# wh-xu/Hyper-Gen

Measured on AMD Instinct MI355X. Metric: genomes/sec sketch (k=21,s=1500,D=4096), higher is better.
Workload: dtype u64

## Files before the change

### hyper-gen_amd/csrc/hg_encode_kernels.hip

```cpp
#include "hg_internal.h"

namespace {

constexpr int ENC_WG = 512;
constexpr int ENC_WAVES = ENC_WG / 64;
constexpr uint64_t WY_INC = 0xa0761d6478bd642full;
constexpr uint64_t WY_XOR = 0xe7037ed1a0b428dbull;

__device__ __forceinline__ uint64_t wy_word(uint64_t hash, uint64_t off) {
  uint64_t s = hash + off;
  unsigned __int128 m = (unsigned __int128)(s ^ WY_XOR) * s;
  return (uint64_t)(m >> 64) ^ (uint64_t)m;
}

__device__ __forceinline__ void csa(uint64_t &hi, uint64_t &lo, uint64_t a, uint64_t b, uint64_t c) {
  const uint32_t a0 = (uint32_t)a, a1 = (uint32_t)(a >> 32), b0 = (uint32_t)b, b1 = (uint32_t)(b >> 32);
  const uint32_t c0 = (uint32_t)c, c1 = (uint32_t)(c >> 32);
  const uint32_t h0 = __builtin_amdgcn_bitop3_b32(a0, b0, c0, 0xE8), h1 = __builtin_amdgcn_bitop3_b32(a1, b1, c1, 0xE8);
  const uint32_t l0 = __builtin_amdgcn_bitop3_b32(a0, b0, c0, 0x96), l1 = __builtin_amdgcn_bitop3_b32(a1, b1, c1, 0x96);
  hi = (uint64_t)h0 | ((uint64_t)h1 << 32);
  lo = (uint64_t)l0 | ((uint64_t)l1 << 32);
}

__device__ __forceinline__ uint64_t harley_seal16(uint64_t *pl, const uint64_t (&x)[16]) {
  uint64_t twosA, twosB, foursA, foursB, eightsA, eightsB, sixteens;
  csa(twosA, pl[0], pl[0], x[0], x[1]);
  csa(twosB, pl[0], pl[0], x[2], x[3]);
  csa(foursA, pl[1], pl[1], twosA, twosB);
  csa(twosA, pl[0], pl[0], x[4], x[5]);
  csa(twosB, pl[0], pl[0], x[6], x[7]);
  csa(foursB, pl[1], pl[1], twosA, twosB);
  csa(eightsA, pl[2], pl[2], foursA, foursB);
  csa(twosA, pl[0], pl[0], x[8], x[9]);
  csa(twosB, pl[0], pl[0], x[10], x[11]);
  csa(foursA, pl[1], pl[1], twosA, twosB);
  csa(twosA, pl[0], pl[0], x[12], x[13]);
  csa(twosB, pl[0], pl[0], x[14], x[15]);
  csa(foursB, pl[1], pl[1], twosA, twosB);
  csa(eightsB, pl[2], pl[2], foursA, foursB);
  csa(sixteens, pl[3], pl[3], eightsA, eightsB);
  return sixteens;
}

constexpr int HI_PLANES = 10;

template <class CountOf>
__device__ __forceinline__ void write_hv_row(uint32_t hv_d, uint32_t layout, uint32_t n, int16_t *__restrict__ out,
                                             int32_t *__restrict__ norm2, int32_t *s_red, CountOf count_of) {
  const uint32_t tid = threadIdx.x, lane = tid & 63, wave = tid >> 6, d_full = (hv_d / 64) * 64;
  uint32_t acc = 0;
  for (uint32_t d = tid; d < hv_d; d += ENC_WG) {
    uint32_t c = 0;
    if (d < d_full) {
      const uint32_t pos = d & 63;
      c = count_of(d >> 6, (layout == HG_LAYOUT_AVX2) ? (16 * (pos & 3) + (pos >> 2)) : pos);
    }
    const int16_t v = (int16_t)(uint16_t)(2u * c - n);
    out[d] = v;
    acc += (uint32_t)((int32_t)v * (int32_t)v);
  }
#pragma unroll
  for (int o = 32; o > 0; o >>= 1) acc += __shfl_down(acc, o);
  if (lane == 0) s_red[wave] = (int32_t)acc;
  __syncthreads();
  if (tid == 0) {
    uint32_t s = 0;
    for (int w = 0; w < ENC_WAVES; ++w) s += (uint32_t)s_red[w];
    *norm2 = (int32_t)s;
  }
}

template <bool SPLIT>
__global__ __launch_bounds__(ENC_WG) void encode_kernel(
    const hg_genome_meta *__restrict__ meta, const uint64_t *__restrict__ hits,
    const uint32_t *__restrict__ ndistinct, uint32_t hv_d, uint32_t layout,
    int16_t *__restrict__ hv_out, int32_t *__restrict__ norm2_out, uint32_t split_over,
    const uint2 *__restrict__ items, uint32_t *__restrict__ accum, uint32_t wave_max) {
  extern __shared__ __attribute__((aligned(16))) uint32_t s_cnt[];
  __shared__ int32_t s_red[ENC_WAVES];
  const uint32_t g = SPLIT ? items[blockIdx.x].x : blockIdx.x;
  const hg_genome_meta gm = meta[g];
  const uint32_t n_all = ndistinct[g];
  if (!SPLIT && (n_all > split_over || n_all <= wave_max || n_all == HG_NHASH_PENDING)) return;
  const uint32_t slab = SPLIT ? (items[blockIdx.x].y & 0xffffu) : 0u, slot = SPLIT ? (items[blockIdx.x].y >> 16) : 0u;
  const uint32_t h0 = SPLIT ? slab * HG_ENC_SLAB : 0u;
  if (SPLIT && h0 >= n_all) return;
  const uint32_t n = SPLIT ? (n_all - h0 < HG_ENC_SLAB ? n_all - h0 : HG_ENC_SLAB) : n_all;
  const uint64_t *__restrict__ hs = hits + gm.hit_off + h0;
  const uint32_t n_words = hv_d / 64;
  const uint32_t stride = n_words + 1;
  const uint32_t tid = threadIdx.x, lane = tid & 63;
  const uint32_t wave = __builtin_amdgcn_readfirstlane(tid >> 6);

  for (uint32_t i = tid; i < 64 * stride; i += ENC_WG) s_cnt[i] = 0;
  __syncthreads();

  const uint32_t n_groups = (n_words + 63) / 64;
  const uint32_t slices = (n_groups == 0 || n_groups >= (uint32_t)ENC_WAVES) ? 1u : (uint32_t)ENC_WAVES / n_groups;
  for (uint32_t job = wave; job < n_groups * slices; job += ENC_WAVES) {
    const uint32_t grp = job / slices, slice = job % slices;
    const uint32_t w = grp * 64 + lane;
    const bool w_ok = w < n_words;
    const uint64_t off = (uint64_t)(w + 1) * WY_INC;
    uint64_t pl[4 + HI_PLANES];
#pragma unroll
    for (int p = 0; p < 4 + HI_PLANES; ++p) pl[p] = 0;
    uint32_t blocks_in_window = 0;

    auto flush = [&]() {
      if (w_ok) {
#pragma unroll 4
        for (uint32_t j = 0; j < 64; ++j) {
          uint32_t c = 0;
#pragma unroll
          for (int p = 0; p < 4 + HI_PLANES; ++p) c |= (uint32_t)((pl[p] >> j) & 1) << p;
          if (c) atomicAdd(&s_cnt[j * stride + w], c);
        }
      }
#pragma unroll
      for (int p = 0; p < 4 + HI_PLANES; ++p) pl[p] = 0;
      blocks_in_window = 0;
    };

    for (uint32_t b0 = slice * 16; b0 < n; b0 += slices * 16) {
      uint64_t x[16];
#pragma unroll
      for (int t = 0; t < 16; ++t) {
        const uint32_t idx = b0 + t;
        x[t] = (idx < n) ? wy_word(hs[idx], off) : 0ull;
      }
      uint64_t carry = harley_seal16(pl, x);
#pragma unroll
      for (int p = 0; p < HI_PLANES; ++p) {
        uint64_t t = pl[4 + p] & carry;
        pl[4 + p] ^= carry;
        carry = t;
      }
      if (++blocks_in_window == (1u << HI_PLANES) - 1) flush();
    }
    flush();
  }
  __syncthreads();

  if (SPLIT) {
    uint32_t *__restrict__ a = accum + (size_t)slot * hv_d;
    for (uint32_t i = tid; i < n_words * 64; i += ENC_WG) {
      const uint32_t w = i >> 6, j = i & 63, c = s_cnt[j * stride + w];
      if (c) atomicAdd(&a[i], c);
    }
    return;
  }
  write_hv_row(hv_d, layout, n, hv_out + (size_t)g * hv_d, norm2_out + g, s_red,
               [&](uint32_t w, uint32_t j) { return s_cnt[j * stride + w]; });
}

typedef short short2v __attribute__((ext_vector_type(2)));

template <int P>
__device__ __forceinline__ void expand_pairs_avx2(const uint64_t *pl, uint32_t n, uint32_t (&packed)[32], uint32_t &acc) {
  const short2v nv = {(short)(uint16_t)n, (short)(uint16_t)n};
#pragma unroll
  for (int m = 0; m < 32; ++m) {
    uint32_t c = 0;
#pragma unroll
    for (int k = 0; k < P; ++k) {
      const int t = m >> 1;
      const uint32_t xw = (m & 1) ? (uint32_t)(pl[k] >> 32) : (uint32_t)pl[k];
      const uint32_t sh = t >= k ? xw >> (t - k) : xw << (k - t);
      c |= sh & (0x00010001u << k);
    }
    const short2v cv = __builtin_bit_cast(short2v, c), v = cv + cv - nv;
    acc = (uint32_t)__builtin_amdgcn_sdot2(v, v, (int)acc, false);
    packed[m] = __builtin_bit_cast(uint32_t, v);
  }
}

__global__ __launch_bounds__(256) void encode_wave_kernel(
    const hg_genome_meta *__restrict__ meta, const uint64_t *__restrict__ hits,
    const uint32_t *__restrict__ ndistinct, uint32_t n_genomes, uint32_t hv_d, uint32_t layout,
    int16_t *__restrict__ hv_out, int32_t *__restrict__ norm2_out, uint32_t wave_max) {
  const uint32_t lane = threadIdx.x & 63;
  const uint32_t g = __builtin_amdgcn_readfirstlane(blockIdx.x * 4 + (threadIdx.x >> 6));
  if (g >= n_genomes) return;
  const uint32_t n = ndistinct[g];
  if (n > wave_max) return;
  const uint64_t *__restrict__ hs = hits + meta[g].hit_off;
  const uint32_t n_words = hv_d / 64;
  int16_t *__restrict__ out = hv_out + (size_t)g * hv_d;
  const bool vec_ok = (hv_d % 8 == 0) && ((reinterpret_cast<uintptr_t>(hv_out) & 15) == 0);
  __shared__ uint4 s_rows[4][512];
  uint4 *const s_row = s_rows[threadIdx.x >> 6];
  const bool via_lds = vec_ok && n < 16 && layout == HG_LAYOUT_AVX2;
  uint32_t acc = 0;
  for (uint32_t grp = 0; grp * 64 < n_words; ++grp) {
    const uint32_t w = grp * 64 + lane;
    const uint64_t off = (uint64_t)(w + 1) * WY_INC;
    uint64_t pl[4 + HI_PLANES];
#pragma unroll
    for (int p = 0; p < 4 + HI_PLANES; ++p) pl[p] = 0;
    for (uint32_t b0 = 0; b0 < n; b0 += 16) {
      uint64_t h[16], x[16];
#pragma unroll
      for (int t = 0; t < 16; ++t) h[t] = hs[b0 + t < n ? b0 + t : n - 1];
#pragma unroll
      for (int t = 0; t < 16; ++t) x[t] = (b0 + t < n) ? wy_word(h[t], off) : 0ull;
      const uint64_t sixteens = harley_seal16(pl, x);
      if (n >= 16) {
        uint64_t carry = sixteens;
#pragma unroll
        for (int p = 0; p < HI_PLANES; ++p) {
          const uint64_t t = pl[4 + p] & carry;
          pl[4 + p] ^= carry;
          carry = t;
        }
      }
    }
    if (via_lds) {
      if (w < n_words) {
        uint32_t packed[32];
        expand_pairs_avx2<4>(pl, n, packed, acc);
#pragma unroll
        for (int q = 0; q < 8; ++q)
          s_row[8 * lane + ((uint32_t)q ^ (lane & 7u))] = make_uint4(packed[4 * q], packed[4 * q + 1], packed[4 * q + 2], packed[4 * q + 3]);
      }
      __builtin_amdgcn_fence(__ATOMIC_RELEASE, "wavefront");
      __builtin_amdgcn_wave_barrier();
      __builtin_amdgcn_fence(__ATOMIC_ACQUIRE, "wavefront");
      const uint32_t pass_words = n_words - grp * 64 < 64u ? n_words - grp * 64 : 64u;
      uint4 *dst = reinterpret_cast<uint4 *>(out + (size_t)grp * 64 * 64);
#pragma unroll 2
      for (uint32_t sidx = 0; sidx < 8; ++sidx) {
        const uint32_t i = sidx * 64 + lane, l = i >> 3, q = i & 7u;
        if (l < pass_words) {
          typedef uint32_t u32x4 __attribute__((ext_vector_type(4)));
          const uint4 v = s_row[8 * l + (q ^ (l & 7u))];
          __builtin_nontemporal_store(u32x4{v.x, v.y, v.z, v.w}, reinterpret_cast<u32x4 *>(dst + i));
        }
      }
      __builtin_amdgcn_fence(__ATOMIC_RELEASE, "wavefront");
      __builtin_amdgcn_wave_barrier();
    } else if (w < n_words) {
      uint32_t packed[32];
      if (layout == HG_LAYOUT_AVX2) {
        if (n < 16) expand_pairs_avx2<4>(pl, n, packed, acc);
        else if (n < 64) expand_pairs_avx2<6>(pl, n, packed, acc);
        else if (n < 256) expand_pairs_avx2<8>(pl, n, packed, acc);
        else expand_pairs_avx2<4 + HI_PLANES>(pl, n, packed, acc);
      } else {
#pragma unroll
        for (int p = 0; p < 64; ++p) {
          uint32_t c = 0;
#pragma unroll
          for (int q = 0; q < 4 + HI_PLANES; ++q) c |= (uint32_t)((pl[q] >> p) & 1) << q;
          const int16_t v = (int16_t)(uint16_t)(2u * c - n);
          acc += (uint32_t)((int32_t)v * (int32_t)v);
          if (p & 1) packed[p >> 1] |= (uint32_t)(uint16_t)v << 16;
          else packed[p >> 1] = (uint32_t)(uint16_t)v;
        }
      }
      int16_t *dst = out + (size_t)w * 64;
      if (vec_ok) {
#pragma unroll
        for (int q = 0; q < 8; ++q)
          reinterpret_cast<uint4 *>(dst)[q] = make_uint4(packed[4 * q], packed[4 * q + 1], packed[4 * q + 2], packed[4 * q + 3]);
      } else {
#pragma unroll
        for (int q = 0; q < 32; ++q) dst[2 * q] = (int16_t)(packed[q] & 0xffffu), dst[2 * q + 1] = (int16_t)(packed[q] >> 16);
      }
    }
  }
  for (uint32_t d = n_words * 64 + lane; d < hv_d; d += 64) {
    const int16_t v = (int16_t)(uint16_t)(0u - n);
    out[d] = v;
    acc += (uint32_t)((int32_t)v * (int32_t)v);
  }
#pragma unroll
  for (int o = 32; o > 0; o >>= 1) acc += __shfl_down(acc, o);
  if (lane == 0) norm2_out[g] = (int32_t)acc;
}

__global__ __launch_bounds__(ENC_WG) void encode_finalize_kernel(const uint32_t *__restrict__ genomes,
                                                                 const uint32_t *__restrict__ ndistinct,
                                                                 const uint32_t *__restrict__ accum, uint32_t hv_d,
                                                                 uint32_t layout, int16_t *__restrict__ hv_out,
                                                                 int32_t *__restrict__ norm2_out) {
  __shared__ int32_t s_red[ENC_WAVES];
  const uint32_t g = genomes[blockIdx.x];
  const uint32_t *__restrict__ a = accum + (size_t)blockIdx.x * hv_d;
  write_hv_row(hv_d, layout, ndistinct[g], hv_out + (size_t)g * hv_d, norm2_out + g, s_red,
               [&](uint32_t w, uint32_t j) { return a[w * 64 + j]; });
}

}

static hipError_t encode_attr() {
  static std::atomic<uint64_t> done{0};
  if (attr_done_on_this_device(done, false)) return hipSuccess;
  hipError_t e = hipFuncSetAttribute(reinterpret_cast<const void *>(&encode_kernel<false>),
                                     hipFuncAttributeMaxDynamicSharedMemorySize, 150 * 1024);
  if (e == hipSuccess)
    e = hipFuncSetAttribute(reinterpret_cast<const void *>(&encode_kernel<true>),
                            hipFuncAttributeMaxDynamicSharedMemorySize, 150 * 1024);
  if (e == hipSuccess) attr_done_on_this_device(done, true);
  return e;
}

hipError_t hg_launch_encode(hipStream_t st, const hg_genome_meta *d_meta, uint32_t n_genomes,
                            const uint64_t *d_hits, const uint32_t *d_ndistinct, uint32_t hv_d,
                            uint32_t layout, int16_t *d_hv, int32_t *d_norm2, const hg_encode_split *split,
                            uint32_t max_hashes, std::string *launched) {
  if (n_genomes == 0) return hipSuccess;
  const size_t lds = (size_t)64 * (hv_d / 64 + 1) * sizeof(uint32_t);
  if (lds > 150 * 1024) return hipErrorInvalidValue;
  hipError_t e = encode_attr();
  if (e != hipSuccess) return e;
  const bool sp = split && split->n_items;
  const uint32_t wave_max = n_genomes >= 8192 ? (uint32_t)HG_ENC_WAVE_MAX : 256u;
  hipLaunchKernelGGL(encode_wave_kernel, dim3((n_genomes + 3) / 4), dim3(256), 0, st, d_meta, d_hits, d_ndistinct, n_genomes,
                     hv_d, layout, d_hv, d_norm2, wave_max);
  if ((e = hipGetLastError()) != hipSuccess) return e;
  hg_note_launch(launched, "encode_wave_kernel");
  if (max_hashes > wave_max) {
    hipLaunchKernelGGL(encode_kernel<false>, dim3(n_genomes), dim3(ENC_WG), lds, st, d_meta, d_hits, d_ndistinct, hv_d,
                       layout, d_hv, d_norm2, sp ? (uint32_t)HG_ENC_SLAB : ~0u, (const uint2 *)nullptr, (uint32_t *)nullptr,
                       wave_max);
    if ((e = hipGetLastError()) != hipSuccess) return e;
    hg_note_launch(launched, "encode_kernel<false>");
  }
  if (!sp) return e;
  if ((e = hipMemsetAsync(split->d_accum, 0, (size_t)split->n_genomes * hv_d * sizeof(uint32_t), st)) != hipSuccess) return e;
  hipLaunchKernelGGL(encode_kernel<true>, dim3(split->n_items), dim3(ENC_WG), lds, st, d_meta, d_hits, d_ndistinct, hv_d,
                     layout, d_hv, d_norm2, ~0u, reinterpret_cast<const uint2 *>(split->d_items), split->d_accum, 0u);
  hipLaunchKernelGGL(encode_finalize_kernel, dim3(split->n_genomes), dim3(ENC_WG), 0, st, split->d_genomes, d_ndistinct,
                     split->d_accum, hv_d, layout, d_hv, d_norm2);
  hg_note_launch(launched, "encode_kernel<true>");
  hg_note_launch(launched, "encode_finalize_kernel");
  return hipGetLastError();
}
```

Before: 129,900.

## Restructure encode kernel with slice merging, direct AVX2 output and hand-written 64-bit mulhi

Replaces the 128-bit multiply in the wyhash word with a hand-scheduled 32-bit multiply chain, and computes hash words lazily inside Harley-Seal quads separated by sched barriers. In the block encode kernel, per-slice bit planes are merged through LDS carry-save rounds rather than atomically flushed per window. When a genome fits in one window, AVX2-layout output is written directly from the planes, skipping the LDS count table. It also adds a bounded carry ripple that stops at the current block count, and pins waves_per_eu. The goal is fewer multiply instructions, fewer LDS atomics and fewer passes. The cost is more LDS, extra barriers, and register pressure from 17 planes.

```diff
diff --git a/hyper-gen_amd/csrc/hg_encode_kernels.hip b/hyper-gen_amd/csrc/hg_encode_kernels.hip
--- a/hyper-gen_amd/csrc/hg_encode_kernels.hip
+++ b/hyper-gen_amd/csrc/hg_encode_kernels.hip
@@ -7,10 +7,25 @@
 constexpr uint64_t WY_INC = 0xa0761d6478bd642full;
 constexpr uint64_t WY_XOR = 0xe7037ed1a0b428dbull;
 
+#ifndef HG_WY_HAND
+#define HG_WY_HAND 1
+#endif
 __device__ __forceinline__ uint64_t wy_word(uint64_t hash, uint64_t off) {
-  uint64_t s = hash + off;
-  unsigned __int128 m = (unsigned __int128)(s ^ WY_XOR) * s;
+  const uint64_t s = hash + off, t = s ^ WY_XOR;
+#if HG_WY_HAND
+  const uint32_t s0 = (uint32_t)s, s1 = (uint32_t)(s >> 32), t0 = (uint32_t)t, t1 = (uint32_t)(t >> 32);
+  const uint64_t A = (uint64_t)s0 * t0;
+  const uint64_t T = (uint64_t)s1 * t0 + (A >> 32);
+  uint64_t W, cm;
+  asm("v_mad_u64_u32 %0, %1, %2, %3, %4" : "=v"(W), "=s"(cm) : "v"(s0), "v"(t1), "v"(T));
+  uint32_t c;
+  asm("v_cndmask_b32_e64 %0, 0, 1, %1" : "=v"(c) : "s"(cm));
+  const uint64_t H = (uint64_t)s1 * t1 + ((W >> 32) | ((uint64_t)c << 32));
+  return ((uint64_t)((uint32_t)A ^ (uint32_t)H)) | ((uint64_t)((uint32_t)W ^ (uint32_t)(H >> 32)) << 32);
+#else
+  unsigned __int128 m = (unsigned __int128)t * s;
   return (uint64_t)(m >> 64) ^ (uint64_t)m;
+#endif
 }
 
 __device__ __forceinline__ void csa(uint64_t &hi, uint64_t &lo, uint64_t a, uint64_t b, uint64_t c) {
@@ -22,43 +37,58 @@
   lo = (uint64_t)l0 | ((uint64_t)l1 << 32);
 }
 
-__device__ __forceinline__ uint64_t harley_seal16(uint64_t *pl, const uint64_t (&x)[16]) {
-  uint64_t twosA, twosB, foursA, foursB, eightsA, eightsB, sixteens;
-  csa(twosA, pl[0], pl[0], x[0], x[1]);
-  csa(twosB, pl[0], pl[0], x[2], x[3]);
-  csa(foursA, pl[1], pl[1], twosA, twosB);
-  csa(twosA, pl[0], pl[0], x[4], x[5]);
-  csa(twosB, pl[0], pl[0], x[6], x[7]);
-  csa(foursB, pl[1], pl[1], twosA, twosB);
-  csa(eightsA, pl[2], pl[2], foursA, foursB);
-  csa(twosA, pl[0], pl[0], x[8], x[9]);
-  csa(twosB, pl[0], pl[0], x[10], x[11]);
-  csa(foursA, pl[1], pl[1], twosA, twosB);
-  csa(twosA, pl[0], pl[0], x[12], x[13]);
-  csa(twosB, pl[0], pl[0], x[14], x[15]);
-  csa(foursB, pl[1], pl[1], twosA, twosB);
-  csa(eightsB, pl[2], pl[2], foursA, foursB);
+#ifndef HG_ENC_SCHED_QUADS
+#define HG_ENC_SCHED_QUADS 1
+#endif
+template <class Word>
+__device__ __forceinline__ uint64_t harley_seal16(uint64_t *pl, Word word) {
+  auto quad = [&](int t0) {
+    const uint64_t x0 = word(t0), x1 = word(t0 + 1), x2 = word(t0 + 2), x3 = word(t0 + 3);
+    uint64_t twosA, twosB, fours;
+    csa(twosA, pl[0], pl[0], x0, x1);
+    csa(twosB, pl[0], pl[0], x2, x3);
+    csa(fours, pl[1], pl[1], twosA, twosB);
+#if HG_ENC_SCHED_QUADS
+    __builtin_amdgcn_sched_barrier(0);
+#endif
+    return fours;
+  };
+  uint64_t eightsA, eightsB, sixteens;
+  const uint64_t f0 = quad(0), f1 = quad(4);
+  csa(eightsA, pl[2], pl[2], f0, f1);
+  const uint64_t f2 = quad(8), f3 = quad(12);
+  csa(eightsB, pl[2], pl[2], f2, f3);
   csa(sixteens, pl[3], pl[3], eightsA, eightsB);
   return sixteens;
 }
 
 constexpr int HI_PLANES = 10;
-
-template <class CountOf>
-__device__ __forceinline__ void write_hv_row(uint32_t hv_d, uint32_t layout, uint32_t n, int16_t *__restrict__ out,
-                                             int32_t *__restrict__ norm2, int32_t *s_red, CountOf count_of) {
-  const uint32_t tid = threadIdx.x, lane = tid & 63, wave = tid >> 6, d_full = (hv_d / 64) * 64;
-  uint32_t acc = 0;
-  for (uint32_t d = tid; d < hv_d; d += ENC_WG) {
-    uint32_t c = 0;
-    if (d < d_full) {
-      const uint32_t pos = d & 63;
-      c = count_of(d >> 6, (layout == HG_LAYOUT_AVX2) ? (16 * (pos & 3) + (pos >> 2)) : pos);
-    }
-    const int16_t v = (int16_t)(uint16_t)(2u * c - n);
-    out[d] = v;
-    acc += (uint32_t)((int32_t)v * (int32_t)v);
-  }
+constexpr int ENC_PLANES = 4 + HI_PLANES;
+constexpr uint32_t ENC_WINDOW_BLOCKS = (1u << HI_PLANES) - 1;
+static_assert(ENC_WINDOW_BLOCKS * 16 == HG_ENC_WAVE_MAX, "one window of the planes is what the wave kernel takes");
+
+template <int Q>
+__device__ __forceinline__ void ripple_from(uint64_t *pl, uint64_t carry, uint32_t b) {
+  if constexpr (Q < HI_PLANES) {
+    if (b >= (1u << Q)) {
+      const uint64_t t = pl[4 + Q] & carry;
+      pl[4 + Q] ^= carry;
+      ripple_from<Q + 1>(pl, t, b);
+    }
+  }
+}
+template <bool FULL>
+__device__ __forceinline__ void encode_block16(uint64_t *pl, const uint64_t *__restrict__ hs, uint32_t b0, uint32_t n, uint64_t off,
+                                               uint32_t b, bool ripple) {
+  uint64_t h[16];
+#pragma unroll
+  for (int t = 0; t < 16; ++t) h[t] = hs[FULL || b0 + t < n ? b0 + t : n - 1];
+  const uint64_t carry = harley_seal16(pl, [&](int t) { return (FULL || b0 + t < n) ? wy_word(h[t], off) : 0ull; });
+  if (ripple) ripple_from<0>(pl, carry, b);
+}
+
+__device__ __forceinline__ void write_norm2(uint32_t acc, int32_t *__restrict__ norm2, int32_t *s_red) {
+  const uint32_t tid = threadIdx.x, lane = tid & 63, wave = tid >> 6;
 #pragma unroll
   for (int o = 32; o > 0; o >>= 1) acc += __shfl_down(acc, o);
   if (lane == 0) s_red[wave] = (int32_t)acc;
@@ -70,13 +100,118 @@
   }
 }
 
+template <class CountOf>
+__device__ __forceinline__ void write_hv_row(uint32_t hv_d, uint32_t layout, uint32_t n, int16_t *__restrict__ out,
+                                             int32_t *__restrict__ norm2, int32_t *s_red, CountOf count_of) {
+  const uint32_t tid = threadIdx.x, d_full = (hv_d / 64) * 64;
+  uint32_t acc = 0;
+  for (uint32_t d = tid; d < hv_d; d += ENC_WG) {
+    uint32_t c = 0;
+    if (d < d_full) {
+      const uint32_t pos = d & 63;
+      c = count_of(d >> 6, (layout == HG_LAYOUT_AVX2) ? (16 * (pos & 3) + (pos >> 2)) : pos);
+    }
+    const int16_t v = (int16_t)(uint16_t)(2u * c - n);
+    out[d] = v;
+    acc += (uint32_t)((int32_t)v * (int32_t)v);
+  }
+  write_norm2(acc, norm2, s_red);
+}
+
+typedef short short2v __attribute__((ext_vector_type(2)));
+
+template <int P>
+__device__ __forceinline__ void expand_pairs_avx2(const uint64_t *pl, uint32_t n, uint32_t (&packed)[32], uint32_t &acc) {
+  static_assert(P <= 15, "planes 15 and up do not reach the 16-bit outputs");
+  const short2v nv = {(short)(uint16_t)n, (short)(uint16_t)n};
+#pragma unroll
+  for (int m = 0; m < 32; ++m) {
+    uint32_t c = 0;
+#pragma unroll
+    for (int k = 0; k < P; ++k) {
+      const int t = m >> 1;
+      const uint32_t xw = (m & 1) ? (uint32_t)(pl[k] >> 32) : (uint32_t)pl[k];
+      const uint32_t sh = t >= k ? xw >> (t - k) : xw << (k - t);
+      c |= sh & (0x00010001u << k);
+    }
+    const short2v cv = __builtin_bit_cast(short2v, c), v = cv + cv - nv;
+    acc = (uint32_t)__builtin_amdgcn_sdot2(v, v, (int)acc, false);
+    packed[m] = __builtin_bit_cast(uint32_t, v);
+  }
+}
+template <int P>
+__device__ __forceinline__ uint4 expand_quad_avx2(const uint64_t *pl, uint32_t n, uint32_t q, uint32_t &acc) {
+  static_assert(P <= 15, "planes 15 and up do not reach the 16-bit outputs");
+  const short2v nv = {(short)(uint16_t)n, (short)(uint16_t)n};
+  uint32_t d[4];
+#pragma unroll
+  for (int i = 0; i < 4; ++i) {
+    const uint32_t t = 2 * q + (i >> 1);
+    uint32_t c = 0;
+#pragma unroll
+    for (int k = 0; k < P; ++k) {
+      const uint32_t xw = (i & 1) ? (uint32_t)(pl[k] >> 32) : (uint32_t)pl[k];
+      c |= __builtin_amdgcn_alignbit(xw, xw, (t - k) & 31u) & (0x00010001u << k);
+    }
+    const short2v cv = __builtin_bit_cast(short2v, c), v = cv + cv - nv;
+    acc = (uint32_t)__builtin_amdgcn_sdot2(v, v, (int)acc, false);
+    d[i] = __builtin_bit_cast(uint32_t, v);
+  }
+  return make_uint4(d[0], d[1], d[2], d[3]);
+}
+
+__host__ __device__ inline uint32_t enc_slices(uint32_t hv_d) {
+  const uint32_t n_groups = (hv_d / 64 + 63) / 64;
+  return (n_groups == 0 || n_groups >= (uint32_t)ENC_WAVES) ? 1u : (uint32_t)ENC_WAVES / n_groups;
+}
+constexpr uint32_t ENC_MERGE_PLANES = 60;
+constexpr uint32_t ENC_MERGE_BYTES = ENC_MERGE_PLANES * 64 * sizeof(uint64_t);
+constexpr int ENC_MERGED_PLANES = ENC_PLANES + 3;
+__host__ __device__ inline size_t enc_lds_bytes(uint32_t hv_d) {
+  return (enc_slices(hv_d) > 1 ? ENC_MERGE_BYTES : 0) + (size_t)64 * (hv_d / 64 + 1) * sizeof(uint32_t);
+}
+
+template <int R>
+__device__ __forceinline__ void merge_round(uint64_t *pl, uint64_t *s_pl, uint32_t wave, uint32_t slice, uint32_t lane) {
+  constexpr uint32_t bit = 1u << R;
+  constexpr int NP = ENC_PLANES + R;
+  static_assert((ENC_WAVES >> (R + 1)) * NP <= (int)ENC_MERGE_PLANES, "the parked planes fit");
+  uint64_t *const park = s_pl + (size_t)(wave >> (R + 1)) * NP * 64 + lane;
+  if ((slice & (2 * bit - 1)) == bit) {
+#pragma unroll
+    for (int p = 0; p < NP; ++p) park[p * 64] = pl[p];
+  }
+  __syncthreads();
+  if ((slice & (2 * bit - 1)) == 0) {
+    uint64_t carry = 0;
+#pragma unroll
+    for (int p = 0; p < NP; ++p) csa(carry, pl[p], pl[p], park[p * 64], carry);
+    pl[NP] = carry;
+  }
+  __syncthreads();
+}
+
+template <int P>
+__device__ __forceinline__ void share_planes(uint64_t *pl, uint64_t *share, uint32_t slice, uint32_t pm) {
+  if (slice == 0) {
+#pragma unroll
+    for (int p = 0; p < P; ++p)
+      if ((uint32_t)p < pm) share[p * 64] = pl[p];
+  }
+  __syncthreads();
+  if (slice != 0) {
+#pragma unroll
+    for (int p = 0; p < P; ++p) pl[p] = (uint32_t)p < pm ? share[p * 64] : 0ull;
+  }
+}
+
 template <bool SPLIT>
-__global__ __launch_bounds__(ENC_WG) void encode_kernel(
+__global__ __launch_bounds__(ENC_WG) __attribute__((amdgpu_waves_per_eu(6, 6))) void encode_kernel(
     const hg_genome_meta *__restrict__ meta, const uint64_t *__restrict__ hits,
     const uint32_t *__restrict__ ndistinct, uint32_t hv_d, uint32_t layout,
     int16_t *__restrict__ hv_out, int32_t *__restrict__ norm2_out, uint32_t split_over,
     const uint2 *__restrict__ items, uint32_t *__restrict__ accum, uint32_t wave_max) {
-  extern __shared__ __attribute__((aligned(16))) uint32_t s_cnt[];
+  extern __shared__ __attribute__((aligned(16))) uint32_t s_mem[];
   __shared__ int32_t s_red[ENC_WAVES];
   const uint32_t g = SPLIT ? items[blockIdx.x].x : blockIdx.x;
   const hg_genome_meta gm = meta[g];
@@ -91,57 +226,91 @@
   const uint32_t stride = n_words + 1;
   const uint32_t tid = threadIdx.x, lane = tid & 63;
   const uint32_t wave = __builtin_amdgcn_readfirstlane(tid >> 6);
-
-  for (uint32_t i = tid; i < 64 * stride; i += ENC_WG) s_cnt[i] = 0;
+  const uint32_t n_groups = (n_words + 63) / 64, slices = enc_slices(hv_d), n_jobs = n_groups * slices;
+  uint64_t *const s_pl = reinterpret_cast<uint64_t *>(s_mem);
+  uint32_t *const s_cnt = s_mem + (slices > 1 ? ENC_MERGE_BYTES / sizeof(uint32_t) : 0);
+  const uint32_t n_blocks = (n + 15) / 16, window = ENC_WINDOW_BLOCKS * slices;
+  const uint32_t n_windows = (n_blocks + window - 1) / window;
+  const bool direct = !SPLIT && layout == HG_LAYOUT_AVX2 && n_windows == 1;
+  int16_t *__restrict__ out = hv_out + (size_t)g * hv_d;
+  const bool vec_ok = (hv_d % 8 == 0) && ((reinterpret_cast<uintptr_t>(hv_out) & 15) == 0);
+  uint32_t acc = 0;
+
+  if (!direct) {
+    for (uint32_t i = tid; i < 64 * stride; i += ENC_WG) s_cnt[i] = 0;
+    __syncthreads();
+  }
+  for (uint32_t job0 = 0; job0 < n_jobs; job0 += ENC_WAVES) {
+    const uint32_t job = job0 + wave, grp = job / slices, slice = job % slices;
+    const bool active = job < n_jobs;
+    const uint32_t w = grp * 64 + lane;
+    const bool w_ok = active && w < n_words;
+    const uint64_t off = (uint64_t)(w + 1) * WY_INC;
+    for (uint32_t win = 0; win < n_windows; ++win) {
+      uint64_t pl[ENC_MERGED_PLANES];
+#pragma unroll
+      for (int p = 0; p < ENC_MERGED_PLANES; ++p) pl[p] = 0;
+      if (active) {
+        const uint32_t n_full = n / 16, b_end = (win + 1) * window < n_full ? (win + 1) * window : n_full;
+        uint32_t b = 0;
+        for (uint32_t B = win * window + slice; B < b_end; B += slices) encode_block16<true>(pl, hs, B * 16, n, off, ++b, true);
+        if (n_full < n_blocks && n_full % slices == slice && n_full / window == win)
+          encode_block16<false>(pl, hs, n_full * 16, n, off, ++b, true);
+      }
+      uint32_t lane_m = lane;
+      asm volatile("" : "+v"(lane_m));
+      const uint32_t w_m = grp * 64 + lane_m;
+      if (slices > 1) {
+        merge_round<0>(pl, s_pl, wave, slice, lane_m);
+        if (slices > 2) merge_round<1>(pl, s_pl, wave, slice, lane_m);
+        if (slices > 4) merge_round<2>(pl, s_pl, wave, slice, lane_m);
+        const uint32_t pm = ENC_PLANES + (slices == 2 ? 1 : slices == 4 ? 2 : 3);
+        uint64_t *const share = s_pl + (size_t)grp * pm * 64 + lane_m;
+        if (direct && n < 4096) share_planes<12>(pl, share, slice, pm);
+        else if (direct) share_planes<15>(pl, share, slice, pm);
+        else share_planes<ENC_MERGED_PLANES>(pl, share, slice, pm);
+      }
+      if (direct) {
+        if (w_ok) {
+          const uint32_t q_per = (uint32_t)ENC_WAVES / slices;
+          int16_t *const dst = out + (size_t)w_m * 64;
+          for (uint32_t q = slice * q_per; q < (slice + 1) * q_per; ++q) {
+            const uint4 v = n < 4096 ? expand_quad_avx2<12>(pl, n, q, acc) : expand_quad_avx2<15>(pl, n, q, acc);
+            if (vec_ok) {
+              reinterpret_cast<uint4 *>(dst)[q] = v;
+            } else {
+              const uint32_t d[4] = {v.x, v.y, v.z, v.w};
+#pragma unroll
+              for (int i = 0; i < 4; ++i) dst[8 * q + 2 * i] = (int16_t)(d[i] & 0xffffu), dst[8 * q + 2 * i + 1] = (int16_t)(d[i] >> 16);
+            }
+          }
+        }
+      } else {
+        if (w_ok) {
+          const uint32_t c_per = 64u / slices;
+#pragma unroll 1
+          for (uint32_t j = slice * c_per; j < (slice + 1) * c_per; ++j) {
+            uint32_t c = 0;
+#pragma unroll
+            for (int p = 0; p < ENC_MERGED_PLANES; ++p) c |= (uint32_t)((pl[p] >> j) & 1) << p;
+            if (c) s_cnt[j * stride + w_m] += c;
+          }
+        }
+        if (slices > 1 && win + 1 < n_windows) __syncthreads();
+      }
+    }
+  }
+
+  if (direct) {
+    for (uint32_t d = n_words * 64 + threadIdx.x; d < hv_d; d += ENC_WG) {
+      const int16_t v = (int16_t)(uint16_t)(0u - n);
+      out[d] = v;
+      acc += (uint32_t)((int32_t)v * (int32_t)v);
+    }
+    write_norm2(acc, norm2_out + g, s_red);
+    return;
+  }
   __syncthreads();
-
-  const uint32_t n_groups = (n_words + 63) / 64;
-  const uint32_t slices = (n_groups == 0 || n_groups >= (uint32_t)ENC_WAVES) ? 1u : (uint32_t)ENC_WAVES / n_groups;
-  for (uint32_t job = wave; job < n_groups * slices; job += ENC_WAVES) {
-    const uint32_t grp = job / slices, slice = job % slices;
-    const uint32_t w = grp * 64 + lane;
-    const bool w_ok = w < n_words;
-    const uint64_t off = (uint64_t)(w + 1) * WY_INC;
-    uint64_t pl[4 + HI_PLANES];
-#pragma unroll
-    for (int p = 0; p < 4 + HI_PLANES; ++p) pl[p] = 0;
-    uint32_t blocks_in_window = 0;
-
-    auto flush = [&]() {
-      if (w_ok) {
-#pragma unroll 4
-        for (uint32_t j = 0; j < 64; ++j) {
-          uint32_t c = 0;
-#pragma unroll
-          for (int p = 0; p < 4 + HI_PLANES; ++p) c |= (uint32_t)((pl[p] >> j) & 1) << p;
-          if (c) atomicAdd(&s_cnt[j * stride + w], c);
-        }
-      }
-#pragma unroll
-      for (int p = 0; p < 4 + HI_PLANES; ++p) pl[p] = 0;
-      blocks_in_window = 0;
-    };
-
-    for (uint32_t b0 = slice * 16; b0 < n; b0 += slices * 16) {
-      uint64_t x[16];
-#pragma unroll
-      for (int t = 0; t < 16; ++t) {
-        const uint32_t idx = b0 + t;
-        x[t] = (idx < n) ? wy_word(hs[idx], off) : 0ull;
-      }
-      uint64_t carry = harley_seal16(pl, x);
-#pragma unroll
-      for (int p = 0; p < HI_PLANES; ++p) {
-        uint64_t t = pl[4 + p] & carry;
-        pl[4 + p] ^= carry;
-        carry = t;
-      }
-      if (++blocks_in_window == (1u << HI_PLANES) - 1) flush();
-    }
-    flush();
-  }
-  __syncthreads();
-
   if (SPLIT) {
     uint32_t *__restrict__ a = accum + (size_t)slot * hv_d;
     for (uint32_t i = tid; i < n_words * 64; i += ENC_WG) {
@@ -150,29 +319,7 @@
     }
     return;
   }
-  write_hv_row(hv_d, layout, n, hv_out + (size_t)g * hv_d, norm2_out + g, s_red,
-               [&](uint32_t w, uint32_t j) { return s_cnt[j * stride + w]; });
-}
-
-typedef short short2v __attribute__((ext_vector_type(2)));
-
-template <int P>
-__device__ __forceinline__ void expand_pairs_avx2(const uint64_t *pl, uint32_t n, uint32_t (&packed)[32], uint32_t &acc) {
-  const short2v nv = {(short)(uint16_t)n, (short)(uint16_t)n};
-#pragma unroll
-  for (int m = 0; m < 32; ++m) {
-    uint32_t c = 0;
-#pragma unroll
-    for (int k = 0; k < P; ++k) {
-      const int t = m >> 1;
-      const uint32_t xw = (m & 1) ? (uint32_t)(pl[k] >> 32) : (uint32_t)pl[k];
-      const uint32_t sh = t >= k ? xw >> (t - k) : xw << (k - t);
-      c |= sh & (0x00010001u << k);
-    }
-    const short2v cv = __builtin_bit_cast(short2v, c), v = cv + cv - nv;
-    acc = (uint32_t)__builtin_amdgcn_sdot2(v, v, (int)acc, false);
-    packed[m] = __builtin_bit_cast(uint32_t, v);
-  }
+  write_hv_row(hv_d, layout, n, out, norm2_out + g, s_red, [&](uint32_t w, uint32_t j) { return s_cnt[j * stride + w]; });
 }
 
 __global__ __launch_bounds__(256) void encode_wave_kernel(
@@ -198,23 +345,9 @@
     uint64_t pl[4 + HI_PLANES];
 #pragma unroll
     for (int p = 0; p < 4 + HI_PLANES; ++p) pl[p] = 0;
-    for (uint32_t b0 = 0; b0 < n; b0 += 16) {
-      uint64_t h[16], x[16];
-#pragma unroll
-      for (int t = 0; t < 16; ++t) h[t] = hs[b0 + t < n ? b0 + t : n - 1];
-#pragma unroll
-      for (int t = 0; t < 16; ++t) x[t] = (b0 + t < n) ? wy_word(h[t], off) : 0ull;
-      const uint64_t sixteens = harley_seal16(pl, x);
-      if (n >= 16) {
-        uint64_t carry = sixteens;
-#pragma unroll
-        for (int p = 0; p < HI_PLANES; ++p) {
-          const uint64_t t = pl[4 + p] & carry;
-          pl[4 + p] ^= carry;
-          carry = t;
-        }
-      }
-    }
+    uint32_t b = 0, b0 = 0;
+    for (; b0 + 16 <= n; b0 += 16) encode_block16<true>(pl, hs, b0, n, off, ++b, true);
+    if (b0 < n) encode_block16<false>(pl, hs, b0, n, off, ++b, n >= 16);
     if (via_lds) {
       if (w < n_words) {
         uint32_t packed[32];
@@ -310,7 +443,7 @@
                             uint32_t layout, int16_t *d_hv, int32_t *d_norm2, const hg_encode_split *split,
                             uint32_t max_hashes, std::string *launched) {
   if (n_genomes == 0) return hipSuccess;
-  const size_t lds = (size_t)64 * (hv_d / 64 + 1) * sizeof(uint32_t);
+  const size_t lds = enc_lds_bytes(hv_d);
   if (lds > 150 * 1024) return hipErrorInvalidValue;
   hipError_t e = encode_attr();
   if (e != hipSuccess) return e;
```

Result: no change. 131,100, median of 6 (+0.9%).
